# zlogic/matrix-eyes

Hardware: AMD Instinct MI355X
Metric: 1536x1536 depth-maps/sec (higher is better)
Workload: dtype f16; 1 GPU; BASELINE.json configs[1]: single 1536x1536 image, 16-bit MFMA HIP path on 1xMI355X, depth map + FOV head (f16 operands: the fp16 checkpoint bit for bit, 7.1e-4 relative L2 from the fp32 CPU path; bf16 operands measure 1.06e-2, outside north_star's 1e-3); batch_per_gpu=1, images=u8 [B,1536,1536,3] synthetic 'structured' (seed 4321 + rank), resident in HBM, checkpoint=synthetic, seed 2024, exact key set, 951.99 M parameters rounded to fp16, f_norm=FOV head (mod.rs:343-358), weights_broadcast=none (one rank), split_operands=3, launch=eager: one launch per kernel

## Files before the change

include/matrix_eyes_hip_ops.h:

```cpp
#ifndef MATRIX_EYES_HIP_OPS_H
#define MATRIX_EYES_HIP_OPS_H

#include "matrix_eyes_hip.h"

#ifdef __cplusplus
extern "C" {
#endif

enum { ME_ACT_NONE = 0, ME_ACT_GELU = 1, ME_ACT_RELU = 2 };

int32_t me_op_linear(me_ctx* ctx, int32_t M, int32_t N, int32_t K, const void* A16, const void* W16,
                     const float* bias, void* out16, float* out32, int32_t act, int32_t tile_cfg);
int32_t me_op_linear_residual(me_ctx* ctx, int32_t M, int32_t N, int32_t K, const void* A16,
                              const void* W16, const float* bias, const float* gamma, float* x32,
                              int32_t tile_cfg);
int32_t me_op_attention(me_ctx* ctx, const void* qkv16, void* out16, int32_t windows, int32_t tokens,
                        int32_t heads);
int32_t me_op_linear_scaled_cols(me_ctx* ctx, int32_t M, int32_t N, int32_t K, const void* A16, const void* W16,
                                 const float* bias, void* out16, int32_t qcols, float qscale, int32_t tile_cfg);
int32_t me_op_attention_prescaled(me_ctx* ctx, const void* qkv16, void* out16, int32_t windows, int32_t tokens,
                                  int32_t heads);
int32_t me_op_layernorm(me_ctx* ctx, const float* x32, const float* weight, const float* bias,
                        void* y16, float* y32, int64_t rows, int32_t dim, float eps);
int32_t me_op_conv2d(me_ctx* ctx, const void* in16b, int32_t B, int32_t H, int32_t W, int32_t Cin,
                     const void* w16, int32_t Cout, int32_t k, int32_t stride, const float* bias,
                     const float* res32, const float* res32b, float* out32, void* out16,
                     int32_t border16, int32_t act, int32_t act_both, int32_t tile_cfg);
int32_t me_op_head_final(me_ctx* ctx, const void* in16b, int32_t B, int32_t H, int32_t W, int32_t Cin, const void* w16,
                         int32_t Cmid, const float* bias, const float* w2, const float* b2, const float* f_norm,
                         float clamp_lo, float clamp_hi, float* out32, int32_t tile_cfg);
int32_t me_op_conv_transpose2x2(me_ctx* ctx, const void* in16, int32_t B, int32_t H, int32_t W,
                                int32_t Cin, const void* w16, int32_t Cout, const float* bias,
                                float* out32, void* out16, int32_t border16, int32_t tile_cfg);
int32_t me_op_conv2d_forms(me_ctx* ctx, const void* in16b, int32_t B, int32_t H, int32_t W, int32_t Cin,
                           const void* w16, int32_t Cout, int32_t k, int32_t stride, const float* bias,
                           const float* res32, const float* res32b, float* out32, void* out16,
                           int32_t border16, int32_t out16_parts, int32_t act, int32_t act_both, int32_t tile_cfg);
int32_t me_op_linear_split(me_ctx* ctx, int32_t M, int32_t N, int32_t K, const void* A16, const void* W16,
                           const float* bias, void* out16, float* out32, int32_t act, int32_t tile_cfg);
int32_t me_op_conv_transpose2x2_forms(me_ctx* ctx, const void* in16, int32_t B, int32_t H, int32_t W,
                                      int32_t Cin, const void* w16, int32_t Cout, const float* bias,
                                      float* out32, void* out16, int32_t border16, int32_t act16,
                                      int32_t out_split, int32_t pixel_stride, int32_t lo_off, int32_t tile_cfg);
int32_t me_op_patch_embed(me_ctx* ctx, const void* patches16, int32_t windows, int32_t P, int32_t C, const void* W16,
                          const float* bias, const float* pos, float* tokens32, int32_t tile_cfg);
int32_t me_op_bilinear(me_ctx* ctx, const float* src32, void* dst16, int32_t planes, int32_t in_size, int32_t out_size,
                       int32_t align_corners);
int32_t me_op_patchify(me_ctx* ctx, const void* x0, const void* x1, const void* x2, void* patches, int32_t batch,
                       int32_t grid);
int32_t me_op_patchify_windows(me_ctx* ctx, const void* xs16, void* patches, int32_t windows, int32_t grid);
int32_t me_op_cls_rows(me_ctx* ctx, float* tokens, const float* cls, const float* pos, int32_t windows, int32_t tpw,
                       int32_t dim);
int32_t me_op_merge(me_ctx* ctx, const float* src32, const void* src16, void* dst16, int32_t batch, int32_t wpi,
                    int32_t win0, int32_t steps, int32_t padding, int32_t grid, int32_t dim, int32_t split);
int32_t me_op_nchw32_to_nhwc(me_ctx* ctx, const float* src, float* dst32, void* dst16, int32_t batch, int32_t H,
                             int32_t W, int32_t C, int32_t border, int32_t relu16, int32_t split);
int32_t me_op_nhwc16_to_nchw32(me_ctx* ctx, const void* src16, float* dst, int32_t batch, int32_t H, int32_t W,
                               int32_t C, int32_t border, int32_t split);
int32_t me_op_nhwc32_to_nchw32(me_ctx* ctx, const float* src, float* dst, int32_t batch, int32_t H, int32_t W,
                               int32_t C);
int32_t me_op_nhwc32_to_16b(me_ctx* ctx, const float* src, void* dst16b, int32_t batch, int32_t H, int32_t W,
                            int32_t C, int32_t relu);
int32_t me_op_concat_channels(me_ctx* ctx, const void* a16, const void* b16, void* dst16, int64_t pixels, int32_t Ca,
                              int32_t Cb);
int32_t me_op_fov_add(me_ctx* ctx, const float* lin, const float* low, void* dst16b, int32_t batch, int32_t grid,
                      int32_t C, int32_t tpw);
int32_t me_op_fov_final(me_ctx* ctx, const void* x16, const float* w, const float* bias, float* fov_deg, float* f_norm,
                        int32_t batch, int32_t k, int32_t C);
int32_t me_op_quantize_fp8(me_ctx* ctx, const void* src16, int64_t rows, int32_t K, int32_t weight_layout,
                           uint8_t* dst8, uint8_t* scales);
int64_t me_op_scale_index(int64_t row, int32_t kblock, int64_t rows, int32_t weight_layout);
int32_t me_op_layernorm_fp8(me_ctx* ctx, const float* x32, const float* weight, const float* bias, uint8_t* y8,
                            uint8_t* yscale, int64_t rows, int32_t dim, float eps);
int32_t me_op_linear_fp8(me_ctx* ctx, int32_t M, int32_t N, int32_t K, const uint8_t* A8, const uint8_t* a_scale,
                         const uint8_t* W8, const uint8_t* w_scale, const float* bias, void* out16, uint8_t* out8,
                         uint8_t* out8_scale, const float* gamma, float* x32);
int32_t me_op_linear_segments(me_ctx* ctx, int32_t M, int32_t N, int32_t K, const void* A16, int32_t seg1, int32_t seg2,
                              const void* const W16[3], const float* const bias[3], const float* const gamma[3],
                              void* out16, float* x32, int32_t act, int32_t tile_cfg);
int32_t me_op_linear_residual_layernorm(me_ctx* ctx, int32_t M, int32_t N, int32_t K, const void* A16, int32_t seg1,
                                        int32_t seg2, const void* const W16[3], const float* const bias[3],
                                        const float* const gamma[3], const float* const ln_w[3], const float* const ln_b[3],
                                        float eps, float* x32, void* xn16);
int32_t me_op_linear_residual_layernorm_fp8(me_ctx* ctx, int32_t M, int32_t N, int32_t K, const void* A16, int32_t seg1,
                                            int32_t seg2, const void* const W16[3], const float* const bias[3],
                                            const float* const gamma[3], const float* const ln_w[3], const float* const ln_b[3],
                                            float eps, float* x32, uint8_t* xn8, uint8_t* xn_scale);
int32_t me_op_linear_fp8_segments(me_ctx* ctx, int32_t M, int32_t N, int32_t K, const uint8_t* A8, const uint8_t* a_scale,
                                  int32_t seg1, int32_t seg2, const uint8_t* const W8[3], const uint8_t* const w_scale[3],
                                  const float* const bias[3], const float* const gamma[3], void* out16, uint8_t* out8,
                                  uint8_t* out8_scale, float* x32);
int32_t me_op_linear_fp8_residual_layernorm(me_ctx* ctx, int32_t M, int32_t N, int32_t K, const uint8_t* A8, const uint8_t* a_scale,
                                            int32_t seg1, int32_t seg2, const uint8_t* const W8[3], const uint8_t* const w_scale[3],
                                            const float* const bias[3], const float* const gamma[3], const float* const ln_w[3],
                                            const float* const ln_b[3], float eps, float* x32, uint8_t* xn8, uint8_t* xn_scale);
int32_t me_op_attention_fp8(me_ctx* ctx, const void* qkv16, uint8_t* out8, uint8_t* out8_scale, int32_t windows,
                            int32_t tokens, int32_t heads);
int32_t me_op_format_f64(me_ctx* ctx, const double* values, int64_t count, char* text, int32_t stride, int32_t* lengths);
int32_t me_calibrate(me_ctx* ctx, double* out6);
int32_t me_op_cast_to16(me_ctx* ctx, const float* src, void* dst16, int64_t count);
int32_t me_op_cast_to32(me_ctx* ctx, const void* src16, float* dst, int64_t count);
int32_t me_profile_enable(me_ctx* ctx, int32_t on);
int32_t me_profile_report(me_ctx* ctx, char* json, int64_t capacity);
int64_t me_op_lanczos3_table(int32_t len_in, int32_t len_out, int32_t* left, int32_t* count,
// ... 10 lines not shown
```

matrix-eyes_amd/_lib.py:

```python
import ctypes as C
import os

_HERE = os.path.dirname(os.path.abspath(__file__))

ME_OK = 0
ERROR_NAMES = {
    1: "BAD_ARG", 2: "BAD_SHAPE", 3: "MISSING_WEIGHT", 4: "BAD_WEIGHT", 5: "HIP", 6: "RCCL",
    7: "IO", 8: "NOT_READY", 9: "OOM", 10: "OVERFLOW",
}
ME_STATUS_OVERFLOW_16BIT = 1
ME_STATUS_SYNC_TIMEOUT = 2
ME_DTYPE_F16, ME_DTYPE_BF16, ME_DTYPE_FP8 = 0, 1, 2
ME_WEIGHT_F32, ME_WEIGHT_F16, ME_WEIGHT_BF16, ME_WEIGHT_F64 = 0, 1, 2, 3
ME_VIT_PATCH_ENCODER, ME_VIT_IMAGE_ENCODER, ME_VIT_FOV_ENCODER = 0, 1, 2


class MatrixEyesError(RuntimeError):
    def __init__(self, code, message):
        super().__init__(f"ME_ERR_{ERROR_NAMES.get(code, code)}: {message}")
        self.code = code
        self.message = message


class CModelConfig(C.Structure):
    _fields_ = [
        ("grid", C.c_int32), ("embed_dim", C.c_int32), ("num_heads", C.c_int32),
        ("depth", C.c_int32), ("tap_blocks", C.c_int32 * 2), ("enc_dims", C.c_int32 * 4),
        ("dec_dim", C.c_int32), ("head_dims", C.c_int32 * 2), ("ln_eps", C.c_float),
        ("align_corners", C.c_int32), ("split_operands", C.c_int32), ("fp8_linears", C.c_int32),
    ]


PROGRESS_FN = C.CFUNCTYPE(None, C.c_void_p, C.c_float, C.c_char_p)

_vp, _i32, _i64, _f32, _u32 = C.c_void_p, C.c_int32, C.c_int64, C.c_float, C.c_uint32

SIGNATURES = {
    "me_abi_version": (_i32, []),
    "me_default_config": (_i32, [C.POINTER(CModelConfig)]),
    "me_ctx_create": (_i32, [_i32, _i32, C.POINTER(CModelConfig), C.POINTER(_vp)]),
    "me_ctx_destroy": (None, [_vp]),
    "me_last_error": (C.c_char_p, [_vp]),
    "me_ctx_set_progress": (_i32, [_vp, PROGRESS_FN, _vp]),
    "me_ctx_set_stream": (_i32, [_vp, _vp]),
    "me_ctx_synchronize": (_i32, [_vp]),
    "me_status_flags": (_i32, [_vp, C.POINTER(_u32)]),
    "me_ln_fusion_state": (_i32, [_vp, C.POINTER(_i32), C.POINTER(_i32)]),
    "me_ctx_set_output_overlap": (_i32, [_vp, _i32]),
    "me_load_weight": (_i32, [_vp, C.c_char_p, _vp, _i32, C.POINTER(_i64), _i32]),
    "me_expected_weight_count": (_i32, [_vp]),
    "me_expected_weight": (_i32, [_vp, _i32, C.POINTER(C.c_char_p), C.POINTER(_i64), C.POINTER(_i32)]),
    "me_weights_finalize": (_i32, [_vp]),
    "me_load_checkpoint_pt": (_i32, [_vp, C.c_char_p]),
    "me_unused_weight_count": (_i32, [_vp]),
    "me_unused_weight_name": (C.c_char_p, [_vp, _i32]),
    "me_weight_arena_bytes": (_i64, [_vp]),
    "me_weight_arena_ptr": (_vp, [_vp]),
    "me_weights_adopt": (_i32, [_vp]),
    "me_weight_arena_layout": (C.c_uint64, [_vp]),
    "me_rccl_unique_id": (_i32, [_vp]),
    "me_bcast_weights": (_i32, [_vp, _vp, _i32, _i32]),
    "me_preprocess_u8": (_i32, [_vp, _vp, _i32, _vp]),
    "me_vit_forward_features": (_i32, [_vp, _i32, _vp, _i32, C.POINTER(_i32), _i32, _vp, C.POINTER(_vp)]),
    "me_encoder_forward_encodings": (_i32, [_vp, _vp, _i32, C.POINTER(_vp)]),
    "me_decoder_forward": (_i32, [_vp, C.POINTER(_vp), _i32, _vp, _vp]),
    "me_head_forward": (_i32, [_vp, _vp, _i32, _vp]),
    "me_fov_forward": (_i32, [_vp, _vp, _vp, _i32, _vp]),
    "me_extract_depth": (_i32, [_vp, _vp, _i32, _vp, _vp, _vp]),
    "me_extract_depth_u8": (_i32, [_vp, _vp, _i32, _vp, _vp, _vp]),
    "me_ctx_set_graph": (_i32, [_vp, _i32]),
    "me_graph_launch_count": (_i64, [_vp]),
    "me_depth_clamp_minmax": (_i32, [_vp, _vp, _i64, C.POINTER(_f32), C.POINTER(_f32)]),
    "me_depth_clamp_minmax_async": (_i32, [_vp, _vp, _i64, _vp]),
    "me_stereogram": (_i32, [_vp, _vp, _i32, _i32, _f32, _f32, _i32, _i32, _f32, _vp, _vp]),
    "me_stereogram_dev_range": (_i32, [_vp, _vp, _i32, _i32, _vp, _i32, _i32, _f32, _vp, _vp]),
    "me_depthmap_rgb_dev_range": (_i32, [_vp, _vp, _i64, _vp, _vp]),
    "me_depthmap_rgb": (_i32, [_vp, _vp, _i64, _f32, _f32, _vp]),
    "me_resize_lanczos3_rgb8": (_i32, [_vp, _vp, _i32, _i32, _vp, _i32, _i32]),
    "me_depthmap_rgb_resized": (_i32, [_vp, _vp, _i32, _i32, _f32, _f32, _vp, _i32, _i32, _vp]),
    "me_jpeg_info": (_i32, [_vp, _i64, C.POINTER(_i32), C.POINTER(_i32), C.POINTER(_i64), C.POINTER(_i64)]),
    "me_jpeg_decode_rgb8": (_i32, [_vp, _vp, _i64, _i32, _vp, _i32, _i32]),
    "me_jpeg_decode_resized_rgb8": (_i32, [_vp, _vp, _i64, _i32, _vp, _i32, _i32]),
    "me_last_jpeg_timing": (_i32, [_vp, C.POINTER(C.c_double)]),
    "me_png_encode_rgb8": (_i32, [_vp, _vp, _i32, _i32, C.POINTER(_vp), C.POINTER(_i64)]),
    "me_output_png": (_i32, [_vp, _vp, _i32, _i32, C.c_char_p]),
    "me_output_depth_map_png": (_i32, [_vp, _vp, _i32, _i32, _f32, _f32, _vp, _i32, _i32, C.c_char_p]),
    "me_output_stereogram_png": (_i32, [_vp, _vp, _i32, _i32, _f32, _f32, _i32, _i32, _f32, _vp, C.c_char_p]),
    "me_mesh_index": (_i32, [_vp, _vp, _i32, _i32, _vp, C.POINTER(_i64), C.POINTER(_i64), _vp]),
    "me_mesh_vertices": (_i32, [_vp, _vp, _i32, _i32, _vp, _i64, _u32, _u32, _vp, _vp]),
    "me_output_mesh": (_i32, [_vp, _vp, _i32, _i32, _u32, _u32, C.c_char_p, C.c_char_p, _i32, _vp]),
    "me_mesh_obj_text": (_i32, [_vp, _vp, _i32, _i32, _u32, _u32, C.c_char_p, _i32, _vp, C.POINTER(_vp), C.POINTER(_i64)]),
    "me_last_mesh_timing": (_i32, [_vp, C.POINTER(C.c_double), C.POINTER(_i64)]),
    "me_ctx_set_write_behind": (_i32, [_vp, _i32]),
    "me_output_flush": (_i32, [_vp]),
    "me_op_linear": (_i32, [_vp, _i32, _i32, _i32, _vp, _vp, _vp, _vp, _vp, _i32, _i32]),
    "me_op_linear_residual": (_i32, [_vp, _i32, _i32, _i32, _vp, _vp, _vp, _vp, _vp, _i32]),
    "me_op_attention": (_i32, [_vp, _vp, _vp, _i32, _i32, _i32]),
    "me_op_attention_prescaled": (_i32, [_vp, _vp, _vp, _i32, _i32, _i32]),
    "me_op_linear_scaled_cols": (_i32, [_vp, _i32, _i32, _i32, _vp, _vp, _vp, _vp, _i32, _f32, _i32]),
    "me_op_layernorm": (_i32, [_vp, _vp, _vp, _vp, _vp, _vp, _i64, _i32, _f32]),
    "me_op_conv2d": (_i32, [_vp, _vp, _i32, _i32, _i32, _i32, _vp, _i32, _i32, _i32, _vp, _vp, _vp,
                            _vp, _vp, _i32, _i32, _i32, _i32]),
    "me_op_head_final": (_i32, [_vp, _vp, _i32, _i32, _i32, _i32, _vp, _i32, _vp, _vp, _vp, _vp, _f32, _f32, _vp, _i32]),
    "me_op_conv_transpose2x2": (_i32, [_vp, _vp, _i32, _i32, _i32, _i32, _vp, _i32, _vp, _vp, _vp,
                                       _i32, _i32]),
    "me_op_conv2d_forms": (_i32, [_vp, _vp, _i32, _i32, _i32, _i32, _vp, _i32, _i32, _i32, _vp, _vp, _vp,
                                  _vp, _vp, _i32, _i32, _i32, _i32, _i32]),
    "me_op_linear_split": (_i32, [_vp, _i32, _i32, _i32, _vp, _vp, _vp, _vp, _vp, _i32, _i32]),
    "me_op_conv_transpose2x2_forms": (_i32, [_vp, _vp, _i32, _i32, _i32, _i32, _vp, _i32, _vp, _vp, _vp,
                                             _i32, _i32, _i32, _i32, _i32, _i32]),
    "me_op_patch_embed": (_i32, [_vp, _vp, _i32, _i32, _i32, _vp, _vp, _vp, _vp, _i32]),
    "me_op_bilinear": (_i32, [_vp, _vp, _vp, _i32, _i32, _i32, _i32]),
    "me_op_patchify": (_i32, [_vp, _vp, _vp, _vp, _vp, _i32, _i32]),
    "me_op_patchify_windows": (_i32, [_vp, _vp, _vp, _i32, _i32]),
    "me_op_cls_rows": (_i32, [_vp, _vp, _vp, _vp, _i32, _i32, _i32]),
    "me_op_merge": (_i32, [_vp, _vp, _vp, _vp, _i32, _i32, _i32, _i32, _i32, _i32, _i32, _i32]),
    "me_op_nchw32_to_nhwc": (_i32, [_vp, _vp, _vp, _vp, _i32, _i32, _i32, _i32, _i32, _i32, _i32]),
    "me_op_nhwc16_to_nchw32": (_i32, [_vp, _vp, _vp, _i32, _i32, _i32, _i32, _i32, _i32]),
    "me_op_nhwc32_to_nchw32": (_i32, [_vp, _vp, _vp, _i32, _i32, _i32, _i32]),
    "me_op_nhwc32_to_16b": (_i32, [_vp, _vp, _vp, _i32, _i32, _i32, _i32, _i32]),
    "me_op_concat_channels": (_i32, [_vp, _vp, _vp, _vp, _i64, _i32, _i32]),
    "me_op_fov_add": (_i32, [_vp, _vp, _vp, _vp, _i32, _i32, _i32, _i32]),
    "me_op_fov_final": (_i32, [_vp, _vp, _vp, _vp, _vp, _vp, _i32, _i32, _i32]),
    "me_op_quantize_fp8": (_i32, [_vp, _vp, _i64, _i32, _i32, _vp, _vp]),
    "me_op_attention_fp8": (_i32, [_vp, _vp, _vp, _vp, _i32, _i32, _i32]),
    "me_op_scale_index": (_i64, [_i64, _i32, _i64, _i32]),
    "me_op_layernorm_fp8": (_i32, [_vp, _vp, _vp, _vp, _vp, _vp, _i64, _i32, _f32]),
    "me_op_linear_fp8": (_i32, [_vp, _i32, _i32, _i32, _vp, _vp, _vp, _vp, _vp, _vp, _vp, _vp, _vp, _vp]),
    "me_op_linear_fp8_segments": (_i32, [_vp, _i32, _i32, _i32, _vp, _vp, _i32, _i32, C.POINTER(_vp), C.POINTER(_vp),
                                         C.POINTER(_vp), C.POINTER(_vp), _vp, _vp, _vp, _vp]),
    "me_op_linear_segments": (_i32, [_vp, _i32, _i32, _i32, _vp, _i32, _i32, C.POINTER(_vp), C.POINTER(_vp), C.POINTER(_vp),
                                     _vp, _vp, _i32, _i32]),
    "me_op_linear_residual_layernorm": (_i32, [_vp, _i32, _i32, _i32, _vp, _i32, _i32, C.POINTER(_vp), C.POINTER(_vp), C.POINTER(_vp),
                                               C.POINTER(_vp), C.POINTER(_vp), _f32, _vp, _vp]),
    "me_op_linear_residual_layernorm_fp8": (_i32, [_vp, _i32, _i32, _i32, _vp, _i32, _i32, C.POINTER(_vp), C.POINTER(_vp), C.POINTER(_vp),
                                                   C.POINTER(_vp), C.POINTER(_vp), _f32, _vp, _vp, _vp]),
    "me_op_linear_fp8_residual_layernorm": (_i32, [_vp, _i32, _i32, _i32, _vp, _vp, _i32, _i32, C.POINTER(_vp), C.POINTER(_vp),
                                                   C.POINTER(_vp), C.POINTER(_vp), C.POINTER(_vp), C.POINTER(_vp), _f32, _vp, _vp, _vp]),
    "me_op_format_f64": (_i32, [_vp, _vp, _i64, _vp, _i32, _vp]),
    "me_calibrate": (_i32, [_vp, C.POINTER(C.c_double)]),
    "me_op_cast_to16": (_i32, [_vp, _vp, _vp, _i64]),
    "me_op_cast_to32": (_i32, [_vp, _vp, _vp, _i64]),
    "me_profile_enable": (_i32, [_vp, _i32]),
    "me_profile_report": (_i32, [_vp, C.c_char_p, _i64]),
    "me_op_lanczos3_table": (_i64, [_i32, _i32, C.POINTER(_i32), C.POINTER(_i32), C.POINTER(_f32), _i64]),
    "me_op_jpeg_decode_host": (_i32, [_vp, _i64, _vp, _i32, _i32]),
    "me_op_gemm_config_count": (_i32, []),
    "me_op_gemm_config_name": (C.c_char_p, [_i32]),
}

_lib = None


def library_path() -> str:
    return os.environ.get("MATRIX_EYES_HIP_LIB", os.path.join(_HERE, "libmatrixeyes_hip.so"))


def load_library():
    global _lib
    if _lib is not None:
        return _lib
    path = library_path()
    if not os.path.exists(path):
        raise MatrixEyesError(5, f"{path} not found: build it first (__graft_entry__.build()); "
                                 "there is no CPU fallback")
    lib = C.CDLL(path)
    for name, (res, args) in SIGNATURES.items():
        fn = getattr(lib, name)
        fn.restype = res
        fn.argtypes = args
    _lib = lib
    return lib


def check(lib, ctx, rc):
    if rc != ME_OK:
        msg = lib.me_last_error(ctx)
        raise MatrixEyesError(rc, msg.decode("utf-8", "replace") if msg else "")
```

matrix-eyes_amd/csrc/api.hip:

```cpp
#include <cmath>
#include <cstdlib>
#include <cstring>
#include <exception>

#include "../../include/matrix_eyes_hip_ops.h"
#include "../host/image_io.hpp"
#include "model.h"
#include "mx_fp8.h"

using namespace me;

namespace {

thread_local std::string g_create_error;

struct OutBuf {
    void* dev = nullptr;
    void* user = nullptr;
    size_t bytes = 0;
    bool staged = false;
};

OutBuf out_buf(me_ctx* ctx, void* user, size_t bytes, const std::string& name) {
    OutBuf o;
// ... 1033 lines not shown
    const float* d = (const float*)to_device(ctx, depth, nv * 4, "out.depth");
    OutBuf ov = out_buf(ctx, vertex_index, nv * 4, "out.vindex");
    OutBuf of;
    if (faces) of = out_buf(ctx, faces, nt * 3 * 4, "out.faces");
    mesh_index_run(d, width, height, (int32_t*)ov.dev, faces ? (int32_t*)of.dev : nullptr, nvertices,
                   nfaces, site_buf(ctx, "out.mesh.ws", mesh_workspace_bytes(width, height)), ctx->stream);
    finish(ctx, ov);
    if (faces && of.staged) {
        ME_HIP(hipMemcpyAsync(faces, of.dev, (size_t)*nfaces * 12, hipMemcpyDeviceToHost,
                              ctx->stream));
        ME_HIP(hipStreamSynchronize(ctx->stream));
    }
    ME_API_END(ctx)
}

int32_t me_mesh_vertices(me_ctx* ctx, const float* depth, int32_t width, int32_t height,
                         const int32_t* vertex_index, int64_t nvertices, uint32_t original_width,
                         uint32_t original_height, float* uv, float* xyz) {
    ME_API_BEGIN(ctx)
    OutputScope out_scope(ctx, depth);
    ME_CHECK(depth && vertex_index && nvertices >= 0, ME_ERR_BAD_ARG, "me_mesh_vertices: bad argument");
    ME_CHECK(original_width > 0 && original_height > 0, ME_ERR_BAD_ARG, "original size 0");
    const size_t nv = (size_t)width * height;
    const float* d = (const float*)to_device(ctx, depth, nv * 4, "out.depth");
    const int32_t* vi = (const int32_t*)to_device(ctx, vertex_index, nv * 4, "out.vindex");
    const uint32_t mx = original_width > original_height ? original_width : original_height;
    const float xm = (float)original_width / (float)mx, ym = (float)original_height / (float)mx;
    OutBuf ouv, oxyz;
    if (uv) ouv = out_buf(ctx, uv, (size_t)nvertices * 8 + 8, "out.uv");
    if (xyz) oxyz = out_buf(ctx, xyz, (size_t)nvertices * 12 + 12, "out.xyz");
    mesh_vertices_launch(d, width, height, vi, xm, ym, uv ? (float*)ouv.dev : nullptr,
                         xyz ? (float*)oxyz.dev : nullptr, ctx->stream);
    if (uv && ouv.staged) from_device(ctx, uv, ouv.dev, (size_t)nvertices * 8);
    if (xyz && oxyz.staged) from_device(ctx, xyz, oxyz.dev, (size_t)nvertices * 12);
    ME_API_END(ctx)
}

static unsigned long long* g_stamps = nullptr;
extern "C" int32_t me_debug_set_stamps(void* dev_ptr) {
    g_stamps = (unsigned long long*)dev_ptr;
    return ME_OK;
}

int32_t me_op_linear(me_ctx* ctx, int32_t M, int32_t N, int32_t K, const void* A16, const void* W16,
                     const float* bias, void* out16, float* out32, int32_t act, int32_t tile_cfg) {
    ME_API_BEGIN(ctx)
    GemmParams p = GemmParams();
    p.stamps = g_stamps;
    p.M = M, p.N = N, p.K = K, p.A = A16, p.lda = K, p.W = W16, p.bias = bias;
    p.out16 = out16, p.out32 = out32, p.ldc = N, p.act = act;
    gemm_launch(p, A_PLAIN, EPI_STORE, ctx->dtype, ctx->stream, tile_cfg);
    ME_API_END(ctx)
}

int32_t me_op_linear_residual(me_ctx* ctx, int32_t M, int32_t N, int32_t K, const void* A16,
                              const void* W16, const float* bias, const float* gamma, float* x32,
                              int32_t tile_cfg) {
    ME_API_BEGIN(ctx)
    ME_CHECK(bias && gamma && x32, ME_ERR_BAD_ARG, "me_op_linear_residual: null pointer");
    GemmParams p = GemmParams();
    p.stamps = g_stamps;
    p.M = M, p.N = N, p.K = K, p.A = A16, p.lda = K, p.W = W16, p.bias = bias, p.gamma = gamma;
    p.res32 = x32, p.out32 = x32, p.ldc = N;
    gemm_launch(p, A_PLAIN, EPI_RESID_SCALE, ctx->dtype, ctx->stream, tile_cfg);
    ME_API_END(ctx)
}

int32_t me_op_attention(me_ctx* ctx, const void* qkv16, void* out16, int32_t windows, int32_t tokens,
                        int32_t heads) {
    ME_API_BEGIN(ctx)
    ME_CHECK(qkv16 && out16, ME_ERR_BAD_ARG, "me_op_attention: null pointer");
    attention_launch(qkv16, out16, windows, tokens, heads, ctx->dtype, ctx->stream);
    ME_API_END(ctx)
}

int32_t me_op_attention_prescaled(me_ctx* ctx, const void* qkv16, void* out16, int32_t windows, int32_t tokens,
                                  int32_t heads) {
    ME_API_BEGIN(ctx)
    ME_CHECK(qkv16 && out16, ME_ERR_BAD_ARG, "me_op_attention_prescaled: null pointer");
    attention_launch(qkv16, out16, windows, tokens, heads, ctx->dtype, ctx->stream, nullptr, nullptr, nullptr, 0, true);
    ME_API_END(ctx)
}

int32_t me_op_linear_scaled_cols(me_ctx* ctx, int32_t M, int32_t N, int32_t K, const void* A16, const void* W16,
                                 const float* bias, void* out16, int32_t qcols, float qscale, int32_t tile_cfg) {
    ME_API_BEGIN(ctx)
    ME_CHECK(A16 && W16 && bias && out16, ME_ERR_BAD_ARG, "me_op_linear_scaled_cols: null pointer");
    GemmParams p = GemmParams();
    p.clamp_lo = -INFINITY, p.clamp_hi = INFINITY;
    p.M = M, p.N = N, p.K = K, p.A = A16, p.lda = K, p.W = W16, p.bias = bias, p.out16 = out16, p.ldc = N;
    p.qcols = qcols, p.qscale = qscale;
    gemm_launch(p, A_PLAIN, EPI_STORE, ctx->dtype, ctx->stream, tile_cfg);
    ME_API_END(ctx)
}

int32_t me_op_layernorm(me_ctx* ctx, const float* x32, const float* weight, const float* bias,
                        void* y16, float* y32, int64_t rows, int32_t dim, float eps) {
    ME_API_BEGIN(ctx)
    ME_CHECK(x32 && weight && bias && (y16 || y32), ME_ERR_BAD_ARG, "me_op_layernorm: null pointer");
    layernorm_launch(x32, weight, bias, y16, y32, rows, dim, eps, ctx->dtype, ctx->stream);
    ME_API_END(ctx)
}

int32_t me_op_conv2d(me_ctx* ctx, const void* in16b, int32_t B, int32_t H, int32_t W, int32_t Cin,
                     const void* w16, int32_t Cout, int32_t k, int32_t stride, const float* bias,
                     const float* res32, const float* res32b, float* out32, void* out16,
                     int32_t border16, int32_t act, int32_t act_both, int32_t tile_cfg) {
    ME_API_BEGIN(ctx)
    ME_CHECK((k == 1 || k == 3) && (stride == 1 || stride == 2), ME_ERR_BAD_SHAPE,
             "me_op_conv2d: k=%d stride=%d", k, stride);
    GemmParams p = GemmParams();
    const int Ho = H / stride, Wo = W / stride;
    p.M = B * Ho * Wo, p.N = Cout, p.K = k * k * Cin, p.A = in16b;
    p.in_Hp = H + 2, p.in_Wp = W + 2, p.Cin = Cin, p.out_H = Ho, p.out_W = Wo;
    p.KH = k, p.KW = k, p.stride = stride, p.W = w16, p.bias = bias;
    p.res32 = res32, p.res32b = res32b, p.out32 = out32, p.out16 = out16, p.ldc = Cout;
    p.out16_border = border16, p.act = act, p.act16_only = act_both ? 0 : 1;
    gemm_launch(p, A_CONV, EPI_STORE, ctx->dtype, ctx->stream, tile_cfg);
    ME_API_END(ctx)
}

int32_t me_op_head_final(me_ctx* ctx, const void* in16b, int32_t B, int32_t H, int32_t W, int32_t Cin, const void* w16,
                         int32_t Cmid, const float* bias, const float* w2, const float* b2, const float* f_norm,
                         float clamp_lo, float clamp_hi, float* out32, int32_t tile_cfg) {
    ME_API_BEGIN(ctx)
    ME_CHECK(in16b && w16 && bias && w2 && b2 && out32, ME_ERR_BAD_ARG, "me_op_head_final: null pointer");
    ME_CHECK(B > 0 && H > 0 && W > 0 && Cin % 64 == 0 && Cmid > 0 && Cmid <= 32 && Cmid % 4 == 0, ME_ERR_BAD_SHAPE,
             "me_op_head_final: %d x %d x %d, %d -> %d", B, H, W, Cin, Cmid);
    GemmParams p = GemmParams();
    p.M = B * H * W, p.N = Cmid, p.K = 9 * Cin, p.A = in16b;
    p.in_Hp = H + 2, p.in_Wp = W + 2, p.Cin = Cin, p.out_H = H, p.out_W = W;
    p.KH = 3, p.KW = 3, p.stride = 1, p.W = w16, p.bias = bias, p.w2 = w2, p.b2 = b2, p.f_norm = f_norm;
    p.pixels_per_image = H * W, p.out32 = out32, p.clamp_lo = clamp_lo, p.clamp_hi = clamp_hi, p.ldc = Cmid;
    gemm_launch(p, A_CONV, EPI_HEAD_FINAL, ctx->dtype, ctx->stream, tile_cfg);
    ME_API_END(ctx)
}

int32_t me_op_conv_transpose2x2(me_ctx* ctx, const void* in16, int32_t B, int32_t H, int32_t W,
                                int32_t Cin, const void* w16, int32_t Cout, const float* bias,
                                float* out32, void* out16, int32_t border16, int32_t tile_cfg) {
    ME_API_BEGIN(ctx)
    GemmParams p = GemmParams();
    p.M = B * H * W, p.N = 4 * Cout, p.K = Cin, p.A = in16, p.lda = Cin, p.W = w16, p.bias = bias;
    p.out_H = H, p.out_W = W, p.Cout = Cout, p.out32 = out32, p.out16 = out16;
    p.out16_border = border16, p.ldc = Cout;
    gemm_launch(p, A_PLAIN, EPI_CONVT, ctx->dtype, ctx->stream, tile_cfg);
    ME_API_END(ctx)
}

int32_t me_op_conv2d_forms(me_ctx* ctx, const void* in16b, int32_t B, int32_t H, int32_t W, int32_t Cin,
                           const void* w16, int32_t Cout, int32_t k, int32_t stride, const float* bias,
                           const float* res32, const float* res32b, float* out32, void* out16,
                           int32_t border16, int32_t out16_parts, int32_t act, int32_t act_both, int32_t tile_cfg) {
    ME_API_BEGIN(ctx)
    ME_CHECK(in16b && w16 && (out32 || out16), ME_ERR_BAD_ARG, "me_op_conv2d_forms: null pointer");
    ME_CHECK((k == 1 || k == 3) && (stride == 1 || stride == 2) && B > 0 && H > 0 && W > 0 && Cin > 0 && Cout > 0 &&
                 H % stride == 0 && W % stride == 0,
             ME_ERR_BAD_SHAPE, "me_op_conv2d_forms: %d x %d x %d, %d -> %d, k=%d stride=%d", B, H, W, Cin, Cout, k, stride);
    ME_CHECK(out16_parts >= 1 && out16_parts <= 3 && (out16_parts == 1 || out16), ME_ERR_BAD_ARG,
             "me_op_conv2d_forms: out16_parts=%d", out16_parts);
    ME_CHECK(act == ME_ACT_NONE || act == ME_ACT_RELU, ME_ERR_BAD_ARG, "me_op_conv2d_forms: act=%d", act);
    GemmParams p = GemmParams();
    p.clamp_lo = -INFINITY, p.clamp_hi = INFINITY;
    const int Ho = H / stride, Wo = W / stride;
    p.M = B * Ho * Wo, p.N = Cout, p.K = k * k * Cin, p.A = in16b;
    p.in_Hp = H + 2, p.in_Wp = W + 2, p.Cin = Cin, p.out_H = Ho, p.out_W = Wo;
// ... 445 lines not shown
```

matrix-eyes_amd/csrc/attention.hip:

```cpp
#include <type_traits>

#include "common.h"
#include "mx_fp8.h"

namespace me {

namespace {

template <typename T>
struct Mfma32;
template <>
struct Mfma32<f16> {
    typedef f16x8 frag;
    static __device__ __forceinline__ f32x16 run(frag a, frag b, f32x16 c) {
        return __builtin_amdgcn_mfma_f32_32x32x16_f16(a, b, c, 0, 0, 0);
    }
};
template <>
struct Mfma32<bf16> {
    typedef bf16x8 frag;
    static __device__ __forceinline__ f32x16 run(frag a, frag b, f32x16 c) {
        return __builtin_amdgcn_mfma_f32_32x32x16_bf16(a, b, c, 0, 0, 0);
    }
};
// ... 240 lines not shown
            const float m_new = fmaxf(m_run, dot);
            const float alpha = __builtin_amdgcn_exp2f((m_run - m_new) * scale_log2e);
            const float pv = __builtin_amdgcn_exp2f((dot - m_new) * scale_log2e);
            m_run = m_new;
            l_run = l_run * alpha + (h == 0 ? pv : 0.f);
            const float p16 = (float)(T)pv;
#pragma unroll
            for (int d = 0; d < 2; ++d)
#pragma unroll
                for (int g4 = 0; g4 < 4; ++g4) {
                    typedef T v4 __attribute__((ext_vector_type(4)));
                    const v4 vv = *reinterpret_cast<const v4*>(vb + ((4 * d + g4) << 4) + 8 * h);
#pragma unroll
                    for (int e = 0; e < 4; ++e)
                        o[d][4 * g4 + e] = __builtin_fmaf(p16, (float)vv[e], o[d][4 * g4 + e] * alpha);
                }
        }
    } else {
        tile(nkt - 1, std::true_type());
    }

    auto round16 = [](float x) -> T {
        asm volatile("" : "+v"(x));
        return (T)x;
    };
    const float l_tot = l_run + __shfl_xor(l_run, 32);
    const float inv = 1.0f / l_tot;
    const int q = q0 + r;
    if (out8) {
        const int64_t m = row0 + q;
#pragma unroll
        for (int d = 0; d < 2; ++d) {
            float v[16];
            float amax = 0.f;
#pragma unroll
            for (int e = 0; e < 16; ++e) {
                v[e] = (float)round16(o[d][e] * inv);
                amax = fmaxf(amax, fabsf(v[e]));
            }
            amax = fmaxf(amax, __shfl_xor(amax, 32));
            const unsigned sb = mx_scale_byte(amax);
            const float sc = mx_inv_scale(sb);
            if (q < tokens) {
                uint8_t* op = out8 + m * C + head * 64 + d * 32 + 4 * h;
#pragma unroll
                for (int g4 = 0; g4 < 4; ++g4)
                    *reinterpret_cast<unsigned*>(op + 8 * g4) =
                        pack_fp8x4(v[4 * g4] * sc, v[4 * g4 + 1] * sc, v[4 * g4 + 2] * sc, v[4 * g4 + 3] * sc);
                if (h == 0) out8_scale[a_scale_index(m, head * 2 + d, out8_mt)] = (uint8_t)sb;
            }
        }
    } else if (q < tokens) {
        T* op = out + (row0 + q) * C + head * 64 + 4 * h;
#pragma unroll
        for (int d = 0; d < 2; ++d)
#pragma unroll
            for (int g4 = 0; g4 < 4; ++g4) {
                typedef T v4 __attribute__((ext_vector_type(4)));
                v4 v;
#pragma unroll
                for (int e = 0; e < 4; ++e) v[e] = round16(o[d][4 * g4 + e] * inv);
                *reinterpret_cast<v4*>(op + d * 32 + 8 * g4) = v;
            }
    }
#ifdef ME_ATT_STAMPS
    if (g_att_stamps && lane == 0 && blockIdx.x < 4096) {
        ph[6] = __builtin_amdgcn_s_memtime() - t_begin;
        for (int i = 0; i < 7; ++i) g_att_stamps[((size_t)blockIdx.x * 4 + wave) * 8 + i] = ph[i];
        g_att_stamps[((size_t)blockIdx.x * 4 + wave) * 8 + 7] = active ? 1 : 0;
    }
#endif
}



template <typename T, int MINW, bool HALVES>
__global__ __launch_bounds__(256, MINW) void attention2_kernel(const T* __restrict__ qkv, T* __restrict__ out,
                                                               int tokens, int heads, int ngroups,
                                                               RowSegs segs, uint8_t* __restrict__ out8,
                                                               uint8_t* __restrict__ out8_scale, int64_t out8_mt,
                                                               float defer_thr) {
    typedef typename Mfma32<T>::frag frag;
    constexpr int NSLOT = 2;
    __shared__ __attribute__((aligned(16))) char smem[NSLOT * 2 * TILE_BYTES];
    const int tid = threadIdx.x, lane = tid & 63;
    const int bid = blockIdx.x;
#ifdef ME_ATT_STAMPS
    unsigned long long ph[8] = {0, 0, 0, 0, 0, 0, 0, 0};
    const unsigned long long t_begin = __builtin_amdgcn_s_memtime();
    unsigned long long t_last = t_begin;
#endif
    const int wave = __builtin_amdgcn_readfirstlane(tid >> 6);
    const int r = lane & 31, h = lane >> 5;
    const int C = heads * 64;
    const int ldq = 3 * C;
    const int nqb = (tokens + 127) >> 7;
    const int xcd = bid & 7, slot0 = bid >> 3;
    const int group = xcd + 8 * (slot0 / nqb);
    const int qblk = slot0 - (slot0 / nqb) * nqb;
    if (group >= ngroups) return;
    const int win = group / heads, head = group - win * heads;
    const int q0 = qblk * 128 + wave * 32;
    int64_t row0 = (int64_t)win * tokens;
    if (segs.seg1 && win >= segs.win0)
        row0 = win < segs.win0 + segs.win1 ? segs.seg1 + (int64_t)(win - segs.win0) * tokens
                                           : segs.seg2 + (int64_t)(win - segs.win0 - segs.win1) * tokens;
    const T* qbase = qkv + head * 64;
    const T* kbase = qkv + C + head * 64;
    const T* vbase = qkv + 2 * C + head * 64;

    const int st_row = lane >> 3, st_slot = lane & 7;
    const unsigned row_bytes = (unsigned)ldq * 2u;
    unsigned koff0, voff0;
    {
        const int rr = (2 * wave) * 8 + st_row;
        koff0 = (unsigned)rr * row_bytes + ((st_slot ^ ((rr >> 1) & 7)) << 4);
        voff0 = (unsigned)rr * row_bytes + ((st_slot ^ (((rr >> 1) & 1) << 2)) << 4);
    }
    const unsigned smem_base = __builtin_amdgcn_readfirstlane(lds_address(smem));
    const char* kwin = uniform_ptr((const char*)(kbase + row0 * ldq));
    const char* vwin = uniform_ptr((const char*)(vbase + row0 * ldq));
    const int nkt = (tokens + KT - 1) / KT;
    auto stage = [&](int kt, int slot) {
        const unsigned dst = smem_base + slot * (2 * TILE_BYTES) + (2 * wave) * 1024;
        const char* kt_k = uniform_ptr(kwin + (size_t)kt * KT * row_bytes);
        const char* kt_v = uniform_ptr(vwin + (size_t)kt * KT * row_bytes);
        if ((kt + 1) * KT <= tokens) {
            unsigned k0 = koff0, v0 = voff0;
            asm volatile("" : "+v"(k0), "+v"(v0));
            glds16_raw(kt_k, k0, dst);
            glds16_raw(kt_v, v0, dst + TILE_BYTES);
            glds16_raw(kt_k, (k0 ^ 64u) + 8u * row_bytes, dst + 1024);
            glds16_raw(kt_v, v0 + 8u * row_bytes, dst + TILE_BYTES + 1024);
        } else {
            const int last = tokens - 1 - kt * KT;
#pragma unroll
            for (int i = 0; i < 2; ++i) {
                const int rr = (2 * wave + i) * 8 + st_row;
                const unsigned rowb = (unsigned)(rr < last ? rr : last) * row_bytes;
                glds16_raw(kt_k, rowb + ((st_slot ^ ((rr >> 1) & 7)) << 4), dst + i * 1024);
                glds16_raw(kt_v, rowb + ((st_slot ^ (((rr >> 1) & 1) << 2)) << 4), dst + TILE_BYTES + i * 1024);
            }
        }
    };

    const int il = lane & 15;
    int k_lane, v_lane;
    {
        const int k_swz = (r >> 1) & 7;
        k_lane = r * 128 + ((h ^ k_swz) << 4);
        const int v_qrow = il >> 2, v_p = il & 3, v_dhalf = (lane >> 4) & 1;
        v_lane = (4 * h + v_qrow) * 128 + ((2 * v_dhalf + (v_p >> 1)) << 4) + ((v_p & 1) << 3) + (((v_qrow >> 1) & 1) << 6);
    }
    f32x16 o[2], lsum, negm;
    o[0] = f32x16{0};
    o[1] = f32x16{0};
    lsum = f32x16{0};
    negm = f32x16{0};
    float m_run = 0.f;
    float l_run = 0.f;
    frag ones;
#pragma unroll
    for (int j = 0; j < 8; ++j) ones[j] = (T)1.0f;

    stage(0, 0);

    frag qf[4];
    {
        int q = q0 + r;
        q = q < tokens ? q : tokens - 1;
        const T* qp = qbase + (row0 + q) * ldq + 8 * h;
#pragma unroll
        for (int s = 0; s < 4; ++s) qf[s] = *reinterpret_cast<const frag*>(qp + 16 * s);
        typedef int i32x4 __attribute__((ext_vector_type(4)));
#pragma unroll
        for (int s = 0; s < 4; ++s) {
            i32x4 t = __builtin_bit_cast(i32x4, qf[s]);
            asm volatile("" : "+v"(t));
            qf[s] = __builtin_bit_cast(frag, t);
        }
    }

    const bool active = q0 < tokens;
    int slot = 0;
    auto tile = [&](int kt, auto first_tag, auto tail_tag) {
        constexpr bool FIRST = decltype(first_tag)::value;
        constexpr bool TAIL = decltype(tail_tag)::value;
#ifdef ME_ATT_STAMPS
        if (FIRST) ph[7] = __builtin_amdgcn_s_memtime() - t_begin;
        t_last = __builtin_amdgcn_s_memtime();
#endif
#ifdef ME_ATT_STAMPS
        const int abl = __builtin_amdgcn_readfirstlane(g_att_mode);
        if (!(abl & 1) || FIRST) {
#endif
        wait_vmcnt<0>();
        __builtin_amdgcn_s_barrier();
        asm volatile("" ::: "memory");
        ATT_PH(0);
        if (kt + 1 < nkt) stage(kt + 1, slot ^ 1);
#ifdef ME_ATT_STAMPS
        }
#endif
        ATT_PH(1);
        unsigned ka = smem_base + slot * (2 * TILE_BYTES) + (unsigned)k_lane;
        unsigned va = smem_base + slot * (2 * TILE_BYTES) + TILE_BYTES + (unsigned)v_lane;
        asm volatile("" : "+v"(ka), "+v"(va));
        slot ^= 1;

        auto part = [&](auto k0_tag, auto nks_tag, bool first_part) {
            constexpr int K0 = decltype(k0_tag)::value, NKS = decltype(nks_tag)::value;
            f32x16 s[NKS];
#ifdef ME_ATT_STAMPS
            if (abl & 8) {
                for (int ks = 0; ks < NKS; ++ks) s[ks] = negm;
                asm volatile("" : "+v"(s[0]), "+v"(s[NKS - 1]));
            } else
#endif
#pragma unroll
            for (int ks = 0; ks < NKS; ++ks) {
#pragma unroll
                for (int st = 0; st < 4; ++st) {
                    const frag kf = lds_read_frag<frag>((ka ^ (unsigned)(st << 5)) + (K0 + ks) * 32 * 128);
                    s[ks] = Mfma32<T>::run(kf, qf[st], st == 0 ? negm : s[ks]);
                }
            }
#ifdef ME_ATT_STAMPS
            asm volatile("" : "+v"(s[0]), "+v"(s[NKS - 1]));
#endif
            ATT_PH(2);
            float mloc = -INFINITY;
#pragma unroll
            for (int ks = 0; ks < NKS; ++ks)
#pragma unroll
                for (int g = 0; g < 16; ++g) {
                    if (TAIL) {
                        const int key = kt * KT + (K0 + ks) * 32 + (g & 3) + 8 * (g >> 2) + 4 * h;
                        if (key >= tokens) s[ks][g] = -INFINITY;
                    }
                    mloc = fmaxf(mloc, s[ks][g]);
                }
            {
                float a = mloc, b = mloc;
                asm volatile("s_nop 1\n\tv_permlane32_swap_b32 %0, %1\n\ts_nop 0" : "+v"(a), "+v"(b));
                mloc = fmaxf(a, b);
            }
            if ((FIRST && first_part) || __any(mloc > defer_thr)) {
                const float delta = (FIRST && first_part) ? mloc : fmaxf(mloc, 0.f);
                if (!(FIRST && first_part)) {
                    const float alpha = __builtin_amdgcn_exp2f(-delta);
#pragma unroll
                    for (int g = 0; g < 16; ++g) o[0][g] *= alpha, o[1][g] *= alpha;
                    if constexpr (HALVES) {
                        l_run *= alpha;
                    } else {
#pragma unroll
                        for (int g = 0; g < 16; ++g) lsum[g] *= alpha;
                    }
                }
                m_run += delta;
#pragma unroll
                for (int g = 0; g < 16; ++g) negm[g] = -m_run;
#pragma unroll
                for (int ks = 0; ks < NKS; ++ks)
#pragma unroll
                    for (int g = 0; g < 16; ++g) s[ks][g] -= delta;
            }
            ATT_PH(3);
#ifdef ME_ATT_STAMPS
            if (!(abl & 2))
#endif
#pragma unroll
            for (int ks = 0; ks < NKS; ++ks)
#pragma unroll
                for (int g = 0; g < 16; ++g) s[ks][g] = __builtin_amdgcn_exp2f(s[ks][g]);

#ifdef ME_ATT_STAMPS
            asm volatile("" : "+v"(s[0]), "+v"(s[NKS - 1]));
#endif
            ATT_PH(4);
#ifdef ME_ATT_STAMPS
            if (abl & 4) {
                asm volatile("" : "+v"(s[0]), "+v"(s[NKS - 1]));
            } else
#endif
#pragma unroll
            for (int ks = 0; ks < NKS; ++ks)
#pragma unroll
                for (int s2 = 0; s2 < 2; ++s2) {
                    frag pf;
#pragma unroll
                    for (int j = 0; j < 8; ++j) pf[j] = (T)s[ks][8 * s2 + j];
                    if constexpr (HALVES) {
#pragma unroll
                        for (int j = 0; j < 8; ++j) l_run += s[ks][8 * s2 + j];
                    } else {
                        lsum = Mfma32<T>::run(ones, pf, lsum);
                    }
#pragma unroll
                    for (int d = 0; d < 2; ++d) {
                        const unsigned vp = (va ^ (unsigned)(d << 6)) + ((K0 + ks) * 32 + 16 * s2) * 128;
                        const s16x4 half0 = lds_read_tr16_at(vp), half1 = lds_read_tr16_at(vp + 8 * 128);
                        typedef short s16x8 __attribute__((__vector_size__(16)));
                        const s16x8 both = __builtin_shufflevector(half0, half1, 0, 1, 2, 3, 4, 5, 6, 7);
                        o[d] = Mfma32<T>::run(__builtin_bit_cast(frag, both), pf, o[d]);
                    }
                }
        };
        if (active) {
            if constexpr (HALVES) {
                part(std::integral_constant<int, 0>(), std::integral_constant<int, 1>(), true);
                part(std::integral_constant<int, 1>(), std::integral_constant<int, 1>(), false);
            } else {
                part(std::integral_constant<int, 0>(), std::integral_constant<int, 2>(), true);
            }
        }
        asm volatile("s_waitcnt lgkmcnt(0)" ::: "memory");
#ifdef ME_ATT_STAMPS
        asm volatile("" : "+v"(o[0]), "+v"(o[1]), "+v"(lsum));
#endif
        ATT_PH(5);
    };
    float l_tot;
    const bool tail_key = (tokens % KT) == 1 && nkt >= 2;
    const int nfull = tail_key ? nkt - 1 : nkt;
    if (nfull == 1) {
        tile(0, std::true_type(), std::true_type());
    } else {
        tile(0, std::true_type(), std::false_type());
        for (int kt = 1; kt + 1 < nfull; ++kt) tile(kt, std::false_type(), std::false_type());
        if (tail_key)
            tile(nfull - 1, std::false_type(), std::false_type());
        else
            tile(nfull - 1, std::false_type(), std::true_type());
    }
    if constexpr (HALVES) l_tot = l_run + __shfl_xor(l_run, 32);
    else l_tot = lsum[0];
    if (tail_key) {
        wait_vmcnt<0>();
        __builtin_amdgcn_s_barrier();
        asm volatile("" ::: "memory");
        if (active) {
            const char* kb = smem + slot * (2 * TILE_BYTES);
            const char* vb = kb + TILE_BYTES;
            float dot = 0.f;
#pragma unroll
            for (int st = 0; st < 4; ++st) {
                const frag kf = *reinterpret_cast<const frag*>(kb + ((2 * st + h) << 4));
#pragma unroll
                for (int j = 0; j < 8; ++j) dot = __builtin_fmaf((float)kf[j], (float)qf[st][j], dot);
            }
            dot += __shfl_xor(dot, 32);
            const float rel = dot - m_run;
            const float delta = fmaxf(rel, 0.f);
            const float alpha = __builtin_amdgcn_exp2f(-delta);
            const float p16 = (float)(T)__builtin_amdgcn_exp2f(rel - delta);
            l_tot = l_tot * alpha + p16;
#pragma unroll
            for (int d = 0; d < 2; ++d)
#pragma unroll
                for (int g4 = 0; g4 < 4; ++g4) {
                    typedef T v4 __attribute__((ext_vector_type(4)));
                    const v4 vv = *reinterpret_cast<const v4*>(vb + ((4 * d + g4) << 4) + 8 * h);
#pragma unroll
                    for (int e = 0; e < 4; ++e)
                        o[d][4 * g4 + e] = __builtin_fmaf(p16, (float)vv[e], o[d][4 * g4 + e] * alpha);
                }
        }
    }

    auto round16 = [](float x) -> T {
        asm volatile("" : "+v"(x));
        return (T)x;
    };
    const float inv = 1.0f / l_tot;
    const int q = q0 + r;
    if (out8) {
        const int64_t m = row0 + q;
#pragma unroll
        for (int d = 0; d < 2; ++d) {
            float v[16];
            float amax = 0.f;
#pragma unroll
            for (int e = 0; e < 16; ++e) {
                v[e] = (float)round16(o[d][e] * inv);
                amax = fmaxf(amax, fabsf(v[e]));
            }
            amax = fmaxf(amax, __shfl_xor(amax, 32));
            const unsigned sb = mx_scale_byte(amax);
            const float sc = mx_inv_scale(sb);
            if (q < tokens) {
                uint8_t* op = out8 + m * C + head * 64 + d * 32 + 4 * h;
#pragma unroll
                for (int g4 = 0; g4 < 4; ++g4)
                    *reinterpret_cast<unsigned*>(op + 8 * g4) =
                        pack_fp8x4(v[4 * g4] * sc, v[4 * g4 + 1] * sc, v[4 * g4 + 2] * sc, v[4 * g4 + 3] * sc);
                if (h == 0) out8_scale[a_scale_index(m, head * 2 + d, out8_mt)] = (uint8_t)sb;
            }
        }
    } else if (q < tokens) {
        T* op = out + (row0 + q) * C + head * 64 + 4 * h;
#pragma unroll
        for (int d = 0; d < 2; ++d)
#pragma unroll
            for (int g4 = 0; g4 < 4; ++g4) {
                typedef T v4 __attribute__((ext_vector_type(4)));
                v4 v;
#pragma unroll
                for (int e = 0; e < 4; ++e) v[e] = round16(o[d][4 * g4 + e] * inv);
                *reinterpret_cast<v4*>(op + d * 32 + 8 * g4) = v;
            }
    }
#ifdef ME_ATT_STAMPS
    if (g_att_stamps && lane == 0 && bid < 4096) {
        ph[6] = __builtin_amdgcn_s_memtime() - t_begin;
        for (int i = 0; i < 7; ++i) g_att_stamps[((size_t)bid * 4 + wave) * 8 + i] = ph[i];
        g_att_stamps[((size_t)bid * 4 + wave) * 8 + 7] = active ? (ph[7] ? ph[7] : 1) : 0;
    }
#endif
}


template <typename T, int MINW>
__global__ __launch_bounds__(256, MINW) void attention2p_kernel(const T* __restrict__ qkv, T* __restrict__ out, int tokens, int heads,
                                                             int ngroups, RowSegs segs, uint8_t* __restrict__ out8,
                                                             uint8_t* __restrict__ out8_scale, int64_t out8_mt, float defer_thr) {
    typedef typename Mfma32<T>::frag frag;
    constexpr int NSLOT = 3;
    __shared__ __attribute__((aligned(16))) char smem[NSLOT * 2 * TILE_BYTES];
    const int tid = threadIdx.x, lane = tid & 63;
    const int bid = blockIdx.x;
    const int wave = __builtin_amdgcn_readfirstlane(tid >> 6);
    const int r = lane & 31, h = lane >> 5;
    const int C = heads * 64;
    const int ldq = 3 * C;
    const int nqb = (tokens + 127) >> 7;
    const int xcd = bid & 7, slot0 = bid >> 3;
    const int group = xcd + 8 * (slot0 / nqb);
    const int qblk = slot0 - (slot0 / nqb) * nqb;
    if (group >= ngroups) return;
    const int win = group / heads, head = group - win * heads;
    const int q0 = qblk * 128 + wave * 32;
    int64_t row0 = (int64_t)win * tokens;
    if (segs.seg1 && win >= segs.win0)
        row0 = win < segs.win0 + segs.win1 ? segs.seg1 + (int64_t)(win - segs.win0) * tokens
                                           : segs.seg2 + (int64_t)(win - segs.win0 - segs.win1) * tokens;
    const T* qbase = qkv + head * 64;
    const T* kbase = qkv + C + head * 64;
    const T* vbase = qkv + 2 * C + head * 64;
    const int st_row = lane >> 3, st_slot = lane & 7;
    const unsigned row_bytes = (unsigned)ldq * 2u;
    unsigned koff0, voff0;
    {
        const int rr = (2 * wave) * 8 + st_row;
        koff0 = (unsigned)rr * row_bytes + ((st_slot ^ ((rr >> 1) & 7)) << 4);
        voff0 = (unsigned)rr * row_bytes + ((st_slot ^ (((rr >> 1) & 1) << 2)) << 4);
    }
    const unsigned smem_base = __builtin_amdgcn_readfirstlane(lds_address(smem));
    const char* kwin = uniform_ptr((const char*)(kbase + row0 * ldq));
    const char* vwin = uniform_ptr((const char*)(vbase + row0 * ldq));
    const int nkt = (tokens + KT - 1) / KT;
    auto stage = [&](int kt, int slot) {
        const unsigned dst = smem_base + slot * (2 * TILE_BYTES) + (2 * wave) * 1024;
        const char* kt_k = uniform_ptr(kwin + (size_t)kt * KT * row_bytes);
        const char* kt_v = uniform_ptr(vwin + (size_t)kt * KT * row_bytes);
        if ((kt + 1) * KT <= tokens) {
            unsigned k0 = koff0, v0 = voff0;
            asm volatile("" : "+v"(k0), "+v"(v0));
            glds16_raw(kt_k, k0, dst);
            glds16_raw(kt_v, v0, dst + TILE_BYTES);
            glds16_raw(kt_k, (k0 ^ 64u) + 8u * row_bytes, dst + 1024);
            glds16_raw(kt_v, v0 + 8u * row_bytes, dst + TILE_BYTES + 1024);
        } else {
            const int last = tokens - 1 - kt * KT;
            int sr = st_row, ss = st_slot;
            asm volatile("" : "+v"(sr), "+v"(ss));
#pragma unroll
            for (int i = 0; i < 2; ++i) {
                const int rr = (2 * wave + i) * 8 + sr;
                const unsigned rowb = (unsigned)(rr < last ? rr : last) * row_bytes;
                glds16_raw(kt_k, rowb + ((ss ^ ((rr >> 1) & 7)) << 4), dst + i * 1024);
                glds16_raw(kt_v, rowb + ((ss ^ (((rr >> 1) & 1) << 2)) << 4), dst + TILE_BYTES + i * 1024);
            }
        }
    };
    const int il = lane & 15;
    int k_lane, v_lane;
    {
        const int k_swz = (r >> 1) & 7;
        k_lane = r * 128 + ((h ^ k_swz) << 4);
        const int v_qrow = il >> 2, v_p = il & 3, v_dhalf = (lane >> 4) & 1;
        v_lane = (4 * h + v_qrow) * 128 + ((2 * v_dhalf + (v_p >> 1)) << 4) + ((v_p & 1) << 3) + (((v_qrow >> 1) & 1) << 6);
    }
    f32x16 o[2], lsum, negm;
// ... 290 lines not shown
```

Baseline: 45.06 depth-maps/s.

## Stage single tail key separately and stage attention output through LDS for coalesced stores

The attention kernel now loads the lone tail key row into a small dedicated LDS region at startup, so the last full tile no longer needs a separate stage plus barrier before the tail-key update. The output epilogue writes each wave's 32x64 result tile into swizzled shared memory and reads it back so each lane stores full 16-byte rows, aiming for coalesced global writes. Tail masking is simplified to a per-subtile valid-count comparison. A segmented prescaled-attention API entry point is also exposed. Risks are extra LDS use and reuse of the K/V slot for output staging, which could reduce occupancy or race if another wave still reads that slot.

```diff
diff --git a/include/matrix_eyes_hip_ops.h b/include/matrix_eyes_hip_ops.h
--- a/include/matrix_eyes_hip_ops.h
+++ b/include/matrix_eyes_hip_ops.h
@@ -20,6 +20,8 @@
                                  const float* bias, void* out16, int32_t qcols, float qscale, int32_t tile_cfg);
 int32_t me_op_attention_prescaled(me_ctx* ctx, const void* qkv16, void* out16, int32_t windows, int32_t tokens,
                                   int32_t heads);
+int32_t me_op_attention_prescaled_segments(me_ctx* ctx, const void* qkv16, void* out16, int32_t windows, int32_t tokens,
+                                           int32_t heads, int64_t seg1, int64_t seg2, int32_t win0, int32_t win1);
 int32_t me_op_layernorm(me_ctx* ctx, const float* x32, const float* weight, const float* bias,
                         void* y16, float* y32, int64_t rows, int32_t dim, float eps);
 int32_t me_op_conv2d(me_ctx* ctx, const void* in16b, int32_t B, int32_t H, int32_t W, int32_t Cin,
diff --git a/matrix-eyes_amd/_lib.py b/matrix-eyes_amd/_lib.py
--- a/matrix-eyes_amd/_lib.py
+++ b/matrix-eyes_amd/_lib.py
@@ -97,6 +97,7 @@
     "me_op_linear_residual": (_i32, [_vp, _i32, _i32, _i32, _vp, _vp, _vp, _vp, _vp, _i32]),
     "me_op_attention": (_i32, [_vp, _vp, _vp, _i32, _i32, _i32]),
     "me_op_attention_prescaled": (_i32, [_vp, _vp, _vp, _i32, _i32, _i32]),
+    "me_op_attention_prescaled_segments": (_i32, [_vp, _vp, _vp, _i32, _i32, _i32, _i64, _i64, _i32, _i32]),
     "me_op_linear_scaled_cols": (_i32, [_vp, _i32, _i32, _i32, _vp, _vp, _vp, _vp, _i32, _f32, _i32]),
     "me_op_layernorm": (_i32, [_vp, _vp, _vp, _vp, _vp, _vp, _i64, _i32, _f32]),
     "me_op_conv2d": (_i32, [_vp, _vp, _i32, _i32, _i32, _i32, _vp, _i32, _i32, _i32, _vp, _vp, _vp,
diff --git a/matrix-eyes_amd/csrc/api.hip b/matrix-eyes_amd/csrc/api.hip
--- a/matrix-eyes_amd/csrc/api.hip
+++ b/matrix-eyes_amd/csrc/api.hip
@@ -1139,6 +1139,19 @@
     ME_API_END(ctx)
 }
 
+int32_t me_op_attention_prescaled_segments(me_ctx* ctx, const void* qkv16, void* out16, int32_t windows, int32_t tokens,
+                                           int32_t heads, int64_t seg1, int64_t seg2, int32_t win0, int32_t win1) {
+    ME_API_BEGIN(ctx)
+    ME_CHECK(qkv16 && out16, ME_ERR_BAD_ARG, "me_op_attention_prescaled_segments: null pointer");
+    ME_CHECK(seg1 >= 0 && seg2 >= seg1 && win0 >= 0 && win1 >= 0 && win0 + win1 <= windows, ME_ERR_BAD_ARG,
+             "me_op_attention_prescaled_segments: segments %lld / %lld, windows %d + %d of %d", (long long)seg1, (long long)seg2,
+             win0, win1, windows);
+    RowSegs segs;
+    segs.seg1 = seg1, segs.seg2 = seg2, segs.win0 = win0, segs.win1 = win1;
+    attention_launch(qkv16, out16, windows, tokens, heads, ctx->dtype, ctx->stream, &segs, nullptr, nullptr, 0, true);
+    ME_API_END(ctx)
+}
+
 int32_t me_op_linear_scaled_cols(me_ctx* ctx, int32_t M, int32_t N, int32_t K, const void* A16, const void* W16,
                                  const float* bias, void* out16, int32_t qcols, float qscale, int32_t tile_cfg) {
     ME_API_BEGIN(ctx)
diff --git a/matrix-eyes_amd/csrc/attention.hip b/matrix-eyes_amd/csrc/attention.hip
--- a/matrix-eyes_amd/csrc/attention.hip
+++ b/matrix-eyes_amd/csrc/attention.hip
@@ -346,7 +346,8 @@
                                                                float defer_thr) {
     typedef typename Mfma32<T>::frag frag;
     constexpr int NSLOT = 2;
-    __shared__ __attribute__((aligned(16))) char smem[NSLOT * 2 * TILE_BYTES];
+    constexpr int TAIL_OFF = NSLOT * 2 * TILE_BYTES;
+    __shared__ __attribute__((aligned(16))) char smem[TAIL_OFF + 1024];
     const int tid = threadIdx.x, lane = tid & 63;
     const int bid = blockIdx.x;
 #ifdef ME_ATT_STAMPS
@@ -385,6 +386,8 @@
     const char* kwin = uniform_ptr((const char*)(kbase + row0 * ldq));
     const char* vwin = uniform_ptr((const char*)(vbase + row0 * ldq));
     const int nkt = (tokens + KT - 1) / KT;
+    const bool tail_key = (tokens % KT) == 1 && nkt >= 2;
+    const int nfull = tail_key ? nkt - 1 : nkt;
     auto stage = [&](int kt, int slot) {
         const unsigned dst = smem_base + slot * (2 * TILE_BYTES) + (2 * wave) * 1024;
         const char* kt_k = uniform_ptr(kwin + (size_t)kt * KT * row_bytes);
@@ -428,6 +431,10 @@
     for (int j = 0; j < 8; ++j) ones[j] = (T)1.0f;
 
     stage(0, 0);
+    if (tail_key && wave == 0) {
+        const char* last_row = uniform_ptr(kwin + (size_t)(tokens - 1) * row_bytes);
+        glds16_raw(last_row, (unsigned)((lane & 7) << 4) + (unsigned)((lane >> 3) & 1) * (unsigned)(2 * C), smem_base + TAIL_OFF);
+    }
 
     frag qf[4];
     {
@@ -462,7 +469,7 @@
         __builtin_amdgcn_s_barrier();
         asm volatile("" ::: "memory");
         ATT_PH(0);
-        if (kt + 1 < nkt) stage(kt + 1, slot ^ 1);
+        if (kt + 1 < nfull) stage(kt + 1, slot ^ 1);
 #ifdef ME_ATT_STAMPS
         }
 #endif
@@ -495,15 +502,22 @@
             ATT_PH(2);
             float mloc = -INFINITY;
 #pragma unroll
-            for (int ks = 0; ks < NKS; ++ks)
+            for (int ks = 0; ks < NKS; ++ks) {
+                int nvalid = 0;
+                if (TAIL) {
+                    nvalid = tokens - kt * KT - (K0 + ks) * 32 - 4 * h;
+                    float s0 = s[ks][0];
+                    asm volatile("" : "+v"(nvalid), "+v"(s0));
+                    s[ks][0] = s0;
+                }
 #pragma unroll
                 for (int g = 0; g < 16; ++g) {
                     if (TAIL) {
-                        const int key = kt * KT + (K0 + ks) * 32 + (g & 3) + 8 * (g >> 2) + 4 * h;
-                        if (key >= tokens) s[ks][g] = -INFINITY;
+                        if ((g & 3) + 8 * (g >> 2) >= nvalid) s[ks][g] = -INFINITY;
                     }
                     mloc = fmaxf(mloc, s[ks][g]);
                 }
+            }
             {
                 float a = mloc, b = mloc;
                 asm volatile("s_nop 1\n\tv_permlane32_swap_b32 %0, %1\n\ts_nop 0" : "+v"(a), "+v"(b));
@@ -586,27 +600,20 @@
         ATT_PH(5);
     };
     float l_tot;
-    const bool tail_key = (tokens % KT) == 1 && nkt >= 2;
-    const int nfull = tail_key ? nkt - 1 : nkt;
     if (nfull == 1) {
         tile(0, std::true_type(), std::true_type());
     } else {
         tile(0, std::true_type(), std::false_type());
-        for (int kt = 1; kt + 1 < nfull; ++kt) tile(kt, std::false_type(), std::false_type());
-        if (tail_key)
-            tile(nfull - 1, std::false_type(), std::false_type());
-        else
-            tile(nfull - 1, std::false_type(), std::true_type());
+        const int nwhole = tail_key ? nfull : nfull - 1;
+        for (int kt = 1; kt < nwhole; ++kt) tile(kt, std::false_type(), std::false_type());
+        if (!tail_key) tile(nfull - 1, std::false_type(), std::true_type());
     }
     if constexpr (HALVES) l_tot = l_run + __shfl_xor(l_run, 32);
     else l_tot = lsum[0];
     if (tail_key) {
-        wait_vmcnt<0>();
-        __builtin_amdgcn_s_barrier();
-        asm volatile("" ::: "memory");
         if (active) {
-            const char* kb = smem + slot * (2 * TILE_BYTES);
-            const char* vb = kb + TILE_BYTES;
+            const char* kb = smem + TAIL_OFF;
+            const char* vb = kb + 128;
             float dot = 0.f;
 #pragma unroll
             for (int st = 0; st < 4; ++st) {
@@ -662,18 +669,36 @@
                 if (h == 0) out8_scale[a_scale_index(m, head * 2 + d, out8_mt)] = (uint8_t)sb;
             }
         }
-    } else if (q < tokens) {
-        T* op = out + (row0 + q) * C + head * 64 + 4 * h;
+    } else if (active) {
+        typedef T v4 __attribute__((ext_vector_type(4)));
+        int ln = lane;
+        asm volatile("" : "+v"(ln));
+        const int r = ln & 31, h = ln >> 5;
+        char* mine = smem + slot * (2 * TILE_BYTES) + wave * 4096;
+        char* wp = mine + r * 128 + ((h ^ (r >> 4)) << 3);
+        const int wswz = (r >> 1) & 7;
 #pragma unroll
         for (int d = 0; d < 2; ++d)
 #pragma unroll
             for (int g4 = 0; g4 < 4; ++g4) {
-                typedef T v4 __attribute__((ext_vector_type(4)));
                 v4 v;
 #pragma unroll
                 for (int e = 0; e < 4; ++e) v[e] = round16(o[d][4 * g4 + e] * inv);
-                *reinterpret_cast<v4*>(op + d * 32 + 8 * g4) = v;
-            }
+                *reinterpret_cast<v4*>(wp + (((4 * d + g4) ^ wswz) << 4)) = v;
+            }
+        asm volatile("s_waitcnt lgkmcnt(0)" ::: "memory");
+        const int rsub = ln >> 3, ch = ln & 7;
+        T* op = out + (row0 + q0 + rsub) * C + head * 64 + 8 * ch;
+        frag rows[4];
+#pragma unroll
+        for (int i = 0; i < 4; ++i)
+            rows[i] = *reinterpret_cast<const frag*>(mine + (8 * i + rsub) * 128 + ((ch ^ (4 * (i & 1) + (rsub >> 1))) << 4));
+        asm volatile("s_waitcnt lgkmcnt(0)" ::: "memory");
+#pragma unroll
+        for (int i = 0; i < 4; ++i) {
+            const frag v = i >= 2 ? __builtin_shufflevector(rows[i], rows[i], 4, 5, 6, 7, 0, 1, 2, 3) : rows[i];
+            if (q0 + 8 * i + rsub < tokens) *reinterpret_cast<frag*>(op + (int64_t)(8 * i) * C) = v;
+        }
     }
 #ifdef ME_ATT_STAMPS
     if (g_att_stamps && lane == 0 && bid < 4096) {
```

Measured after the change: 45.37 depth-maps/s (median of 6 runs). Within noise of the previous version (+0.7%).
